# pyprob/pyprob

Hardware: AMD Instinct MI355X
Metric: ic_train_traces_per_sec (higher is better)
Workload: dtype f32; 1 GPU; GaussianUnknownMean IC training, offline traces resident in HBM, LSTM hidden=512, batch=1024 per GPU; traces_in_hbm=1000000, params=1643583, global_batch=1024, parallelism=dp1, optimizer=Adam lr=1e-3*sqrt(world), launch=one Python iteration per step (ICEngine.train_step), eager launches, prewarm_steps=5470, minibatches_resident=976, minibatch_walk=step i trains minibatch (i * 1) mod 976 of the resident dataset

## Files before the change

pyprob_amd/csrc/kernels.hip:

```cpp
#include "common.hpp"
#include "gather.hpp"
#include "head_math.hpp"
#include "aux_jobs.hpp"

#include <math.h>
#include <stdarg.h>
#include <stdlib.h>

#include <algorithm>
#include <vector>

namespace pp {

static thread_local char g_err[512] = "";
void set_error(const char* fmt, ...) {
    va_list ap;
    va_start(ap, fmt);
    vsnprintf(g_err, sizeof(g_err), fmt, ap);
    va_end(ap);
}
const char* last_error() { return g_err; }

constexpr int COLSUM_ROWS = 64;
constexpr int COLSUM_MAX_JOBS = 48;
// ... 712 lines not shown
    __builtin_amdgcn_fence(__ATOMIC_ACQUIRE, "wavefront");
}

template <int KIND, int NE>
__global__ __launch_bounds__(256) void head_tail_kernel(const TailJobs jobs, int64_t lda1, int hid, int K,
                                                        const float* __restrict__ value,
                                                        const float* __restrict__ prior, int rows_per_wave,
                                                        float grad_scale, float* __restrict__ lp_out, int64_t lddy,
                                                        int64_t lddz, float* __restrict__ loss_acc,
                                                        int32_t* __restrict__ nonfinite, long long* __restrict__ dbg) {
    extern __shared__ __attribute__((aligned(16))) float tail_lds[];
    const TailJob& jb = jobs.j[blockIdx.y];
    const int n = jb.n;
    if ((int)blockIdx.x * 4 * rows_per_wave >= n) return;
    const float* __restrict__ A1 = jb.A1;
    const float* __restrict__ W2 = jb.W2;
    const float* __restrict__ b2 = jb.b2;
    const int32_t* __restrict__ rows = jb.rows;
    float* __restrict__ DY = jb.DY;
    float* __restrict__ dZ1 = jb.dZ1;
#define PP_STAMP(k) do { if (dbg && threadIdx.x == 0 && blockIdx.y == 0 && blockIdx.x == 0) dbg[(k)] = clock64(); } while (0)
    PP_STAMP(0);
    const int tid = threadIdx.x, lane = tid & 63, wave = tid >> 6;
    const int n_out = 3 * K;
    const int hid4 = (hid + 3) & ~3;
    const int ws = hid | 1;
    const int wtot = n_out * ws, wtot4 = (wtot + 3) & ~3;
    float* const w2s = tail_lds;
    float* const a1s = tail_lds + wtot4 + wave * hid4;
    float* const ys = tail_lds + wtot4 + 4 * hid4 + wave * 128;
    float* const dys = ys + 64;
    if (ws == hid && (reinterpret_cast<uintptr_t>(W2) & 15) == 0) {
        const f32x4* __restrict__ src = reinterpret_cast<const f32x4*>(W2);
        const int n4 = wtot >> 2;
        for (int base = tid; base < n4; base += 256 * 8) {
            f32x4 v[8];
#pragma unroll
            for (int u = 0; u < 8; ++u) v[u] = src[min(base + 256 * u, n4 - 1)];
#pragma unroll
            for (int u = 0; u < 8; ++u)
                if (base + 256 * u < n4) *reinterpret_cast<f32x4*>(w2s + 4 * (base + 256 * u)) = v[u];
        }
        for (int i = 4 * n4 + tid; i < wtot; i += 256) w2s[i] = W2[i];
    } else {
        const float inv = 1.0f / (float)ws;
        for (int base = tid; base < wtot; base += 256 * 16) {
            float v[16];
#pragma unroll
            for (int u = 0; u < 16; ++u) {
                const int i = min(base + 256 * u, wtot - 1);
                const int o = (int)(((float)i + 0.5f) * inv);
                const int j = i - o * ws;
                v[u] = W2[o * hid + min(j, hid - 1)];
            }
#pragma unroll
            for (int u = 0; u < 16; ++u)
                if (base + 256 * u < wtot) w2s[base + 256 * u] = v[u];
        }
    }
    const bool comp = lane < K;
    const float b2mu = comp ? b2[lane] : 0.0f, b2sd = comp ? b2[K + lane] : 0.0f, b2z = comp ? b2[2 * K + lane] : 0.0f;
    __syncthreads();
    PP_STAMP(1);
    const bool bwd = DY != nullptr;
    float loss_local = 0.f;
    bool bad_any = false;
    const int half = lane >> 5, l31 = lane & 31;
    const int jh = ((hid + 7) >> 3) << 2;
    const int jbeg = half * jh, jend = min(hid, jbeg + jh);
    int jc[NE];
#pragma unroll
    for (int e = 0; e < NE; ++e) jc[e] = min(lane + 64 * e, hid - 1);
    const int i0 = (blockIdx.x * 4 + wave) * rows_per_wave;
    for (int t = 0; t < rows_per_wave; ++t) {
        const int i = i0 + t;
        if (i >= n) break;
        const int r = rows ? rows[i] : i;
        float a1v[NE];
#pragma unroll
        for (int e = 0; e < NE; ++e) {
            const int j = lane + 64 * e;
            a1v[e] = j < hid ? A1[(int64_t)i * lda1 + j] : 0.0f;
            if (j < hid4) a1s[j] = a1v[e];
        }
        wave_lds_sync();
        PP_STAMP(2);
        for (int ob = 0; ob < n_out; ob += 32) {
            const int o = ob + l31;
            const float* __restrict__ wr = w2s + min(o, n_out - 1) * ws;
            float p0 = 0.0f, p1 = 0.0f, p2 = 0.0f, p3 = 0.0f;
            int j = jbeg;
#pragma unroll 4
            for (; j + 3 < jend; j += 4) {
                const f32x4 av = *reinterpret_cast<const f32x4*>(a1s + j);
                p0 += av[0] * wr[j];
                p1 += av[1] * wr[j + 1];
                p2 += av[2] * wr[j + 2];
                p3 += av[3] * wr[j + 3];
            }
            for (; j < jend; ++j) p0 += a1s[j] * wr[j];
            float acc = (p0 + p1) + (p2 + p3);
            acc += __shfl_xor(acc, 32, 64);
            if (half == 0 && o < n_out) ys[o] = acc;
        }
        wave_lds_sync();
        const float ymu = comp ? ys[lane] + b2mu : 0.0f;
        const float ysd = comp ? ys[K + lane] + b2sd : 0.0f;
        const float yz = comp ? ys[2 * K + lane] + b2z : -INFINITY;
        PP_STAMP(3);
        const float v = value[r], pa = prior[2 * r], pb = prior[2 * r + 1];
        const auto red_sum = [](float x) { return wave_sum(x); };
        const auto red_max = [](float x) { return wave_max(x); };
        LaneMixture hm;
        const float lp = lane_mixture_logprob<KIND>(comp, ymu, ysd, yz, v, pa, pb, red_sum, red_max, hm);
        PP_STAMP(4);
        if (lp_out && lane == 0) lp_out[r] = lp;
        const bool rescued = (lp == -INFINITY);
        const bool bad = !rescued && !isfinite(lp);
        bad_any |= bad;
        if (lane == 0) loss_local += rescued ? -kLogEps : -lp;
        if (!bwd) continue;
        const bool live = !(rescued || bad);
        float d0, d1, d2;
        lane_mixture_grad<KIND>(hm, comp, live, lp, pa, pb, grad_scale, red_sum, d0, d1, d2);
        if (comp) {
            float* dy = DY + (int64_t)i * lddy;
            dy[lane] = d0; dy[K + lane] = d1; dy[2 * K + lane] = d2;
            dys[lane] = d0; dys[K + lane] = d1; dys[2 * K + lane] = d2;
        }
        wave_lds_sync();
        PP_STAMP(5);
        float dz[NE];
#pragma unroll
        for (int e = 0; e < NE; ++e) dz[e] = 0.0f;
#pragma unroll 2
        for (int o = 0; o < n_out; ++o) {
            const float d = dys[o];
            const float* __restrict__ wr = w2s + o * ws;
#pragma unroll
            for (int e = 0; e < NE; ++e) dz[e] += d * wr[jc[e]];
        }
#pragma unroll
        for (int e = 0; e < NE; ++e) {
            const int j = lane + 64 * e;
            if (j < hid4) dZ1[(int64_t)i * lddz + j] = (j < hid && a1v[e] > 0.0f) ? dz[e] : 0.0f;
        }
        wave_lds_sync();
    }
    PP_STAMP(6);
    if (lane == 0 && loss_acc && loss_local != 0.0f) atomicAdd(loss_acc + 32 * ((blockIdx.x * 4 + wave + 7 * blockIdx.y) & 63), loss_local);
    if (bad_any && nonfinite && lane == 0) atomicOr(nonfinite, 1);
}

static size_t head_tail_lds_floats(int hid, int n_out) {
    const int hid4 = (hid + 3) & ~3;
    return (size_t)((n_out * (hid | 1) + 3) & ~3) + 4 * (size_t)hid4 + 4 * 128;
}

bool head_tail_supported(int kind, int hid, int n_out) {
    static const bool disabled = false;
    if (disabled) return false;
    if (kind != PP_HEAD_NORMAL_MIXTURE && kind != PP_HEAD_TRUNCNORMAL_MIXTURE && kind != PP_HEAD_POISSON_TN_MIXTURE) return false;
    if (n_out % 3 != 0 || n_out / 3 > MAXK || n_out / 3 < 1) return false;
    return hid >= 1 && hid <= 1024 && head_tail_lds_floats(hid, n_out) <= TAIL_LDS_FLOATS;
}

long long* g_timeline = nullptr;

template <int KIND, int NE>
static int head_tail_launch_ne(dim3 grid, size_t lds, hipStream_t st, const TailJobs& jobs, int64_t lda1, int hid, int K,
                               const float* value, const float* prior, int rpw, float gs, float* lp_out, int64_t lddy,
                               int64_t lddz, float* loss_acc, int32_t* nonfinite) {
    static thread_local bool configured = false;
    if (!configured) {
        hipError_t e = hipFuncSetAttribute((const void*)head_tail_kernel<KIND, NE>, hipFuncAttributeMaxDynamicSharedMemorySize,
                                           (int)(TAIL_LDS_FLOATS * sizeof(float)));
        if (e != hipSuccess) {
            set_error("head_tail: hipFuncSetAttribute failed: %s", hipGetErrorString(e));
            return (int)e;
        }
        configured = true;
    }
    hipLaunchKernelGGL((head_tail_kernel<KIND, NE>), grid, dim3(256), lds, st, jobs, lda1, hid, K, value, prior, rpw, gs, lp_out,
                       lddy, lddz, loss_acc, nonfinite, g_timeline);
    return 0;
}

template <int KIND>
static int head_tail_launch(int ne, dim3 grid, size_t lds, hipStream_t st, const TailJobs& jobs, int64_t lda1, int hid, int K,
                            const float* value, const float* prior, int rpw, float gs, float* lp_out, int64_t lddy,
                            int64_t lddz, float* loss_acc, int32_t* nonfinite) {
#define PP_TAIL(N) return head_tail_launch_ne<KIND, N>(grid, lds, st, jobs, lda1, hid, K, value, prior, rpw, gs, lp_out, lddy, \
                                                       lddz, loss_acc, nonfinite)
    if (ne <= 2) PP_TAIL(2);
    if (ne <= 4) PP_TAIL(4);
    if (ne <= 6) PP_TAIL(6);
    if (ne <= 8) PP_TAIL(8);
    if (ne <= 12) PP_TAIL(12);
    PP_TAIL(16);
#undef PP_TAIL
}

int head_tail_multi(int kind, const TailJob* jobs, int count, int64_t lda1, int hid, int n_out, const float* value,
                    const float* prior, float grad_scale, float* lp_out, int64_t lddy, int64_t lddz, float* loss_acc,
                    int32_t* nonfinite, hipStream_t st) {
    PP_CHECK_ARG(head_tail_supported(kind, hid, n_out), "head_tail: unsupported head shape");
    PP_CHECK_ARG(lda1 % 4 == 0 && lddz % 4 == 0, "head_tail: leading dimensions must be multiples of 4");
    const int ne = (hid + 63) / 64;
    const size_t lds = head_tail_lds_floats(hid, n_out) * sizeof(float);
    int i = 0;
    while (i < count) {
        TailJobs pack;
        int nj = 0, max_n = 0;
        for (; i < count && nj < TAIL_MAX_JOBS; ++i) {
            if (jobs[i].n <= 0) continue;
            PP_CHECK_ARG(jobs[i].A1 && jobs[i].W2 && jobs[i].b2 && (!jobs[i].DY || jobs[i].dZ1), "head_tail: bad job");
            pack.j[nj++] = jobs[i];
            max_n = std::max(max_n, jobs[i].n);
        }
        if (nj == 0) continue;
        const int rpw = std::max((max_n + 4 * 256 - 1) / (4 * 256), 1);
        dim3 grid(cdiv(max_n, 4 * rpw), nj);
        if (kind == PP_HEAD_NORMAL_MIXTURE)
            PP_TRY(head_tail_launch<0>(ne, grid, lds, st, pack, lda1, hid, n_out / 3, value, prior, rpw, grad_scale, lp_out, lddy,
                                       lddz, loss_acc, nonfinite));
        else if (kind == PP_HEAD_TRUNCNORMAL_MIXTURE)
            PP_TRY(head_tail_launch<1>(ne, grid, lds, st, pack, lda1, hid, n_out / 3, value, prior, rpw, grad_scale, lp_out, lddy,
                                       lddz, loss_acc, nonfinite));
        else
            PP_TRY(head_tail_launch<2>(ne, grid, lds, st, pack, lda1, hid, n_out / 3, value, prior, rpw, grad_scale, lp_out, lddy,
                                       lddz, loss_acc, nonfinite));
        PP_LAUNCH_CHECK("head_tail");
    }
    return 0;
}

__global__ void loss_finalize_kernel(const float* __restrict__ acc, const int32_t* __restrict__ flag, float inv_b,
                                     float* __restrict__ loss_out, int32_t* __restrict__ status_out) {
    float tot = 0.0f;
    for (int k = 0; k < 64; ++k) tot += acc[32 * k];
    const float l = tot * inv_b;
    loss_out[0] = l;
    if (status_out) status_out[0] = (flag[0] != 0 || !isfinite(l)) ? 1 : 0;
}

__global__ __launch_bounds__(256) void loss_rows_kernel(const float* __restrict__ lp, int n_rows, float inv_b,
                                                        const int32_t* __restrict__ flag, float* __restrict__ loss_out,
                                                        int32_t* __restrict__ status_out) {
    __shared__ double part[256];
    __shared__ int bad[256];
    double acc = 0.0;
    int b = 0;
    for (int r = threadIdx.x; r < n_rows; r += 256) {
        float l = lp[r];
        if (l == -INFINITY) l = kLogEps;
        if (!isfinite(l)) b = 1;
        acc -= (double)l;
    }
    part[threadIdx.x] = acc;
    bad[threadIdx.x] = b;
    __syncthreads();
    for (int s = 128; s > 0; s >>= 1) {
        if (threadIdx.x < s) {
            part[threadIdx.x] += part[threadIdx.x + s];
            bad[threadIdx.x] |= bad[threadIdx.x + s];
        }
        __syncthreads();
    }
    if (threadIdx.x == 0) {
        const float l = (float)(part[0] * (double)inv_b);
        loss_out[0] = l;
        if (status_out) status_out[0] = (bad[0] || (flag && flag[0] != 0) || !isfinite(l)) ? 1 : 0;
    }
}

int loss_from_rows(const float* lp, int n_rows, int n_traces, const int32_t* flag, float* loss_out, int32_t* status_out,
                   hipStream_t st) {
    hipLaunchKernelGGL(loss_rows_kernel, dim3(1), dim3(256), 0, st, lp, n_rows, 1.0f / (float)n_traces, flag, loss_out,
                       status_out);
    PP_LAUNCH_CHECK("loss_from_rows");
    return 0;
}

int loss_finalize(const float* acc, const int32_t* flag, int n_traces, float* loss_out, int32_t* status_out,
                  hipStream_t st) {
    hipLaunchKernelGGL(loss_finalize_kernel, dim3(1), dim3(1), 0, st, acc, flag, 1.0f / (float)n_traces, loss_out,
                       status_out);
    PP_LAUNCH_CHECK("loss_finalize");
    return 0;
}

constexpr int ADAM_TOP = 1024, ADAM_FIRST = 1025, ADAM_CHUNKS = 1026;
constexpr int ADAM_SEEN = 1027;

__global__ __launch_bounds__(256) void adam_kernel(float* __restrict__ P, float* __restrict__ Gr, float* __restrict__ M,
                                                   float* __restrict__ V, const int32_t* __restrict__ chunk_tensor,
                                                   int n_chunks, const float* __restrict__ active,
                                                   int32_t* __restrict__ tensor_step, int32_t* __restrict__ scratch, float lr,
                                                   float beta1, float beta2, float eps, float wd, float gscale,
                                                   int zero_grads, const int32_t* __restrict__ skip) {
    __shared__ float s_corr[2];
    const int b = blockIdx.x;
    const bool skipped = skip && skip[0] != 0;
    const int t = chunk_tensor[b];
    if (t < 0 || !(active[t] > 0.0f)) return;
    if (skipped) {
        if (zero_grads) *reinterpret_cast<f32x4*>(Gr + (int64_t)b * 1024 + threadIdx.x * 4) = f32x4{0.f, 0.f, 0.f, 0.f};
        return;
    }
    int32_t* const sc = scratch + (int64_t)t * PP_ADAM_SCRATCH;
    const int64_t o = (int64_t)b * 1024 + threadIdx.x * 4;
    const f32x4 g0 = *reinterpret_cast<const f32x4*>(Gr + o);
    __shared__ int s_seen;
    if (threadIdx.x == 0) s_seen = __atomic_load_n(sc + ADAM_SEEN, __ATOMIC_RELAXED);
    __syncthreads();
    const bool seen = s_seen != 0;
    bool idle = false;
    if (!seen && wd == 0.0f) {
        const bool zero = g0[0] == 0.0f && g0[1] == 0.0f && g0[2] == 0.0f && g0[3] == 0.0f;
        idle = __syncthreads_and(zero ? 1 : 0) != 0;
        if (!idle && threadIdx.x == 0) __atomic_store_n(sc + ADAM_SEEN, 1, __ATOMIC_RELAXED);
    } else if (!seen && threadIdx.x == 0) {
        __atomic_store_n(sc + ADAM_SEEN, 1, __ATOMIC_RELAXED);
    }
    f32x4 p = f32x4{0.f, 0.f, 0.f, 0.f}, m = p, v = p;
    if (!idle) {
        p = *reinterpret_cast<f32x4*>(P + o);
        m = *reinterpret_cast<f32x4*>(M + o);
        v = *reinterpret_cast<f32x4*>(V + o);
    }
    int step_old = 0, first = 0, chunks = 0;
    if (threadIdx.x == 0) {
        first = __atomic_load_n(sc + ADAM_FIRST, __ATOMIC_RELAXED) - 1;
        chunks = __atomic_load_n(sc + ADAM_CHUNKS, __ATOMIC_RELAXED);
        if (first < 0) {
            int lo = 0, hi = b;
            while (lo < hi) {
                const int mid = (lo + hi) >> 1;
                if (chunk_tensor[mid] < t) lo = mid + 1; else hi = mid;
            }
            int lo2 = b, hi2 = n_chunks;
            while (lo2 < hi2) {
                const int mid = (lo2 + hi2) >> 1;
                if (chunk_tensor[mid] <= t) lo2 = mid + 1; else hi2 = mid;
            }
            first = lo;
            chunks = lo2 - lo;
        }
        step_old = __atomic_load_n(tensor_step + t, __ATOMIC_RELAXED);
        const int step = step_old + 1;
        double p1 = 1.0, p2 = 1.0, q1 = (double)beta1, q2 = (double)beta2;
        for (int e = step; e > 0; e >>= 1) {
            if (e & 1) { p1 *= q1; p2 *= q2; }
            q1 *= q1;
            q2 *= q2;
        }
        const double bc1 = 1.0 - p1, bc2 = 1.0 - p2;
        s_corr[0] = (float)((double)lr / bc1);
        s_corr[1] = (float)(1.0 / sqrt(bc2));
    }
    __syncthreads();
    const float step_size = s_corr[0], inv_sqrt_bc2 = s_corr[1];
    const int k = (b - first) & 31;
    const int quota = (chunks - k + 31) >> 5;
    int ticket = -1;
    if (threadIdx.x == 0) ticket = atomicAdd(sc + 32 * k, 1);
    if (!idle) {
#pragma unroll
        for (int e = 0; e < 4; ++e) {
            float g = g0[e] * gscale;
            if (wd != 0.0f) g += wd * p[e];
            m[e] = beta1 * m[e] + (1.0f - beta1) * g;
            v[e] = beta2 * v[e] + (1.0f - beta2) * g * g;
            const float denom = sqrtf(v[e]) * inv_sqrt_bc2 + eps;
            p[e] -= step_size * (m[e] / denom);
        }
        *reinterpret_cast<f32x4*>(P + o) = p;
        *reinterpret_cast<f32x4*>(M + o) = m;
        *reinterpret_cast<f32x4*>(V + o) = v;
        if (zero_grads) *reinterpret_cast<f32x4*>(Gr + o) = f32x4{0.f, 0.f, 0.f, 0.f};
    }
    if (threadIdx.x == 0 && ticket == quota - 1) {
        __atomic_store_n(sc + 32 * k, 0, __ATOMIC_RELAXED);
        if (atomicAdd(sc + ADAM_TOP, 1) == min(chunks, 32) - 1) {
            __atomic_store_n(sc + ADAM_TOP, 0, __ATOMIC_RELAXED);
            __atomic_store_n(sc + ADAM_FIRST, first + 1, __ATOMIC_RELAXED);
            __atomic_store_n(sc + ADAM_CHUNKS, chunks, __ATOMIC_RELAXED);
            __atomic_store_n(tensor_step + t, step_old + 1, __ATOMIC_RELAXED);
        }
    }
}

int adam_step(float* params, float* grads, float* m, float* v, int64_t n_params, const int32_t* chunk_tensor,
              const float* active, int32_t* tensor_step, int32_t* scratch, int n_tensors, float lr, float beta1, float beta2,
              float eps, float wd, float gscale, int flags, const int32_t* skip, hipStream_t st) {
    PP_CHECK_ARG(params && grads && m && v && chunk_tensor && active && tensor_step && scratch, "pp_adam_step: null pointer");
    PP_CHECK_ARG(n_params % 1024 == 0, "pp_adam_step: n_params must be a multiple of 1024 (padded tensors)");
    if (n_tensors <= 0 || n_params == 0) return 0;
    const int n_chunks = (int)(n_params / 1024);
    hipLaunchKernelGGL(adam_kernel, dim3((unsigned)n_chunks), dim3(256), 0, st, params, grads, m, v, chunk_tensor, n_chunks,
                       active, tensor_step, scratch, lr, beta1, beta2, eps, wd, gscale, (flags & PP_ADAM_ZERO_GRADS) ? 1 : 0, skip);
    PP_LAUNCH_CHECK("pp_adam_step");
    return 0;
}

}
```

pyprob_amd/csrc/obs_embed.hip:

```cpp
#include "common.hpp"
#include "gather.hpp"
#include "obs_embed.hpp"
#include "panel.hpp"

#include <stdlib.h>

#include <algorithm>

namespace pp {

template <int NOBS>
__global__ __launch_bounds__(256) void obs_embed_fwd_kernel(const ObsFusedArgs ain, const float* __restrict__ P,
                                                            const float* __restrict__ obs, int n_traces,
                                                            int traces_per_wave, float* __restrict__ cat,
                                                            float* __restrict__ f1, float* __restrict__ E,
                                                            const RowBuild rbin, const AddrBias ab,
                                                            const PanelTranspose tr) {
    __shared__ float lds[10240];
    const ObsFusedArgs a = ain;
    const RowBuild rb = rbin;
    if (tr.n_blocks && (int)blockIdx.x >= tr.first_block) {
        panel_transpose_block(tr, (int)blockIdx.x - tr.first_block, lds);
        return;
    }
    if (ab.AB && (int)blockIdx.x >= ab.first_block) {
        addr_bias_block(ab, (int)blockIdx.x - ab.first_block, lds);
        return;
    }
    warm_kernargs((int)(sizeof(ObsFusedArgs) + sizeof(RowBuild) + sizeof(AddrBias) + sizeof(PanelTranspose)) + 64);
    const int tid = threadIdx.x, lane = tid & 63, wave = tid >> 6;
    if (rb.zero_small && blockIdx.x == 0)
        for (int q = tid; q < rb.n_small; q += 256) rb.zero_small[q] = 0.0f;
    obs_stage_all<NOBS>(a, P, lds, tid);
    __syncthreads();
    const int b0 = (blockIdx.x * 4 + wave) * traces_per_wave;
    for (int t = 0; t < traces_per_wave; ++t) {
        const int b = b0 + t;
        if (b >= n_traces) break;
        float h = 0.0f, c = 0.0f;
        int ci = 0, co = 0;
#pragma unroll
        for (int o = 0; o < NOBS; ++o) {
            if (o >= a.n_obs) break;
            const int jh = lane - a.hoff[o];
            const bool acth = jh >= 0 && jh < a.hid[o];
            if (acth) {
                const float* w = lds + a.l0[o].lds_w + jh * (a.in[o] + 1);
                float s = lds[a.l0[o].lds_b + jh];
                for (int i = 0; i < a.in[o]; ++i) s += w[i] * obs[(int64_t)b * a.width + ci + i];
                h = relu_keep_nan(s);
                a.obs_h[o][(int64_t)b * a.ohid_ld[o] + jh] = h;
            }
            ci += a.in[o];
        }
#pragma unroll
        for (int o = 0; o < NOBS; ++o) {
            if (o >= a.n_obs) break;
            const int jc = lane - co;
            const bool actc = jc >= 0 && jc < a.out[o];
            const float v = obs_dense(lds, a.l1[o], jc, actc, h, a.hoff[o]);
            if (actc) c = v;
            co += a.out[o];
        }
        const bool acte = lane < a.e_obs;
        if (acte) cat[(int64_t)b * a.e_ld + lane] = c;
        const float y1 = obs_dense(lds, a.f0, lane, acte, c, 0);
        if (acte) f1[(int64_t)b * a.e_ld + lane] = y1;
        const float y2 = obs_dense(lds, a.f1, lane, acte, y1, 0);
        if (acte) E[(int64_t)b * a.e_ld + lane] = y2;
        if (rb.X) {
            {
                const int c4 = rb.d.e_obs + rb.d.smp + rb.d.dtype + rb.d.addr;
                const int ad = rb.xcols > c4 ? rb.addr[b] : 0;
                float* xr = rb.X + (int64_t)b * rb.ldx;
                if (acte) xr[lane] = y2;
                for (int c = rb.d.e_obs + lane; c < rb.xcols; c += 64) xr[c] = gather_embedding_elem(rb.d, rb.params, rb.at, c, -1, 0.0f, ad);
                if (rb.zero_like) {
                    float* zr = rb.zero_like + (int64_t)b * rb.ldx;
                    for (int c = lane; c < rb.xcols; c += 64) zr[c] = 0.0f;
                }
            }
            for (int t = 1; t < rb.t_max; ++t) {
                const int r0 = rb.row_off[t];
                if (b >= rb.row_off[t + 1] - r0) break;
                const int r = r0 + b;
                const int pr = rb.prev_row[r];
                const int ap = pr < 0 ? -1 : rb.addr[pr];
                const float v = pr < 0 ? 0.0f : rb.value[pr];
                const int ad = rb.addr[r];
                float* xr = rb.X + (int64_t)r * rb.ldx;
                if (acte) xr[lane] = y2;
                for (int c = rb.d.e_obs + lane; c < rb.xcols; c += 64) xr[c] = gather_embedding_elem(rb.d, rb.params, rb.at, c, ap, v, ad);
                if (rb.zero_like) {
                    float* zr = rb.zero_like + (int64_t)r * rb.ldx;
                    for (int c = lane; c < rb.xcols; c += 64) zr[c] = 0.0f;
                }
            }
        }
    }
}

template <int NOBS>
__global__ __launch_bounds__(256) void obs_embed_dgrad_kernel(const ObsFusedArgs ain, const float* __restrict__ P,
                                                              int n_traces, int traces_per_wave,
                                                              const float* __restrict__ cat, const float* __restrict__ f1,
                                                              const float* __restrict__ dX, int64_t ldx,
                                                              const int32_t* __restrict__ row_off, int t_max,
                                                              const float* __restrict__ E, float* __restrict__ dE,
                                                              float* __restrict__ dF1, float* __restrict__ dCat,
                                                              float* const dHo0, int64_t dh_stride, int n_split,
                                                              int64_t split_stride) {
    __shared__ float lds[10240];
    warm_kernargs((int)sizeof(ObsFusedArgs) + 96);
    const ObsFusedArgs a = ain;
    const int tid = threadIdx.x, lane = tid & 63, wave = tid >> 6;
    int oh = -1, jh = 0;
    const float* my_h = nullptr;
    int64_t my_hld = 0;
#pragma unroll
    for (int o = 0; o < NOBS; ++o)
        if (o < a.n_obs && lane >= a.hoff[o] && lane < a.hoff[o] + a.hid[o]) {
            oh = o; jh = lane - a.hoff[o];
            my_h = a.obs_h[o]; my_hld = a.ohid_ld[o];
        }
    const bool acte = lane < a.e_obs;
    const int b0 = (blockIdx.x * 4 + wave) * traces_per_wave;
    auto load_dz2 = [&](int b) {
        float acc = 0.0f;
        if (acte) {
            acc = dX[(int64_t)b * ldx + lane];
            for (int z0 = 1; z0 < n_split; z0 += 8) {
                float pv[8];
#pragma unroll
                for (int u = 0; u < 8; ++u)
                    pv[u] = (z0 + u < n_split) ? dX[(int64_t)(z0 + u) * split_stride + (int64_t)b * ldx + lane] : 0.0f;
                acc += ((pv[0] + pv[1]) + (pv[2] + pv[3])) + ((pv[4] + pv[5]) + (pv[6] + pv[7]));
            }
            for (int t = 1; t < t_max; ++t) {
                const int r0 = row_off[t];
                if (b >= row_off[t + 1] - r0) break;
                acc += dX[(int64_t)(r0 + b) * ldx + lane];
            }
            acc = E[(int64_t)b * a.e_ld + lane] > 0.0f ? acc : 0.0f;
        }
        return acc;
    };
    float nx_dz2 = 0.f, nx_f1 = 0.f, nx_cat = 0.f, nx_h = 0.f;
    if (b0 < n_traces) {
        nx_dz2 = load_dz2(b0);
        nx_f1 = acte ? f1[(int64_t)b0 * a.e_ld + lane] : 0.0f;
        nx_cat = acte ? cat[(int64_t)b0 * a.e_ld + lane] : 0.0f;
        nx_h = oh >= 0 ? my_h[(int64_t)b0 * my_hld + jh] : 0.0f;
    }
    obs_stage_all<NOBS>(a, P, lds, tid);
    __syncthreads();
    for (int t = 0; t < traces_per_wave; ++t) {
        const int b = b0 + t;
        if (b >= n_traces) break;
        const float dz2 = nx_dz2, f1v = nx_f1, catv = nx_cat, hv = nx_h;
        if (t + 1 < traces_per_wave && b + 1 < n_traces) {
            const int bn = b + 1;
            nx_dz2 = load_dz2(bn);
            nx_f1 = acte ? f1[(int64_t)bn * a.e_ld + lane] : 0.0f;
            nx_cat = acte ? cat[(int64_t)bn * a.e_ld + lane] : 0.0f;
            nx_h = oh >= 0 ? my_h[(int64_t)bn * my_hld + jh] : 0.0f;
        }
        if (acte) dE[(int64_t)b * a.e_ld + lane] = dz2;
        float dz1 = obs_dense_t(lds, a.f1, lane, acte, dz2, 0);
        dz1 = f1v > 0.0f ? dz1 : 0.0f;
        if (acte) dF1[(int64_t)b * a.e_ld + lane] = dz1;
        float dzc = obs_dense_t(lds, a.f0, lane, acte, dz1, 0);
        dzc = catv > 0.0f ? dzc : 0.0f;
        if (acte) dCat[(int64_t)b * a.e_ld + lane] = dzc;
        float dh = 0.0f;
        int co = 0;
#pragma unroll
        for (int o = 0; o < NOBS; ++o) {
            if (o >= a.n_obs) break;
            const bool acth = (oh == o);
            const float d = obs_dense_t(lds, a.l1[o], jh, acth, dzc, co);
            if (acth) dh = d;
            co += a.out[o];
        }
        if (oh >= 0) dHo0[(int64_t)oh * dh_stride + (int64_t)b * my_hld + jh] = hv > 0.0f ? dh : 0.0f;
    }
}

static inline int64_t round4(int64_t x) { return (x + 3) & ~int64_t(3); }

bool obs_fused_supported(const pp_net* net) {
    if (net->e_obs > OBS_EMAX) return false;
    for (int o = 0; o < net->n_obs; ++o)
        if (net->obs_depth[o] != 0 && net->obs_depth[o] != 2) return false;
    int hsum = 0;
    for (int o = 0; o < net->n_obs; ++o) {
        if (net->obs_in[o] > OBS_INMAX || net->obs_hid[o] > OBS_HIDMAX || net->obs_hid[o] < 1) return false;
        hsum += net->obs_hid[o];
    }
    return hsum <= 64;
}

bool obs_fused_args(const pp_net* net, float* const* obs_h, ObsFusedArgs& a) {
    for (int o = 0; o < PP_MAX_OBS; ++o) a.obs_h[o] = o < net->n_obs ? obs_h[o] : nullptr;
    a.n_obs = net->n_obs;
    a.e_obs = net->e_obs;
    a.e_ld = round4(net->e_obs);
    int lds = 0, hoff = 0, width = 0;
    auto layer = [&](ObsLayer& L, int64_t w, int64_t b, int rows, int cols) {
        L.w_off = w; L.b_off = b; L.rows = rows; L.cols = cols;
        L.lds_w = lds; lds += rows * (cols + 1);
        L.lds_b = lds; lds += rows;
    };
    for (int o = 0; o < net->n_obs; ++o) {
        a.in[o] = net->obs_in[o]; a.hid[o] = net->obs_hid[o]; a.out[o] = net->obs_out[o];
        a.hoff[o] = hoff; hoff += a.hid[o];
        a.ohid_ld[o] = round4(a.hid[o]);
        width += a.in[o];
        layer(a.l0[o], net->obs_w0[o], net->obs_b0[o], a.hid[o], a.in[o]);
        layer(a.l1[o], net->obs_w1[o], net->obs_b1[o], a.out[o], a.hid[o]);
    }
    a.width = width;
    layer(a.f0, net->fin_w0, net->fin_b0, net->e_obs, net->e_obs);
    layer(a.f1, net->fin_w1, net->fin_b1, net->e_obs, net->e_obs);
    a.lds_total = lds;
    return lds + 1 <= 10240;
}

static int pick_traces_per_wave(int n, int target_blocks) {
    return std::max((n + 4 * target_blocks - 1) / (4 * target_blocks), 1);
}

int obs_embed_fwd_fused(const pp_net* net, const float* P, const float* obs, int n_traces, float* const* obs_h,
                        float* cat, float* f1, float* E, hipStream_t st, const RowBuild* rows, const AddrBias* bias,
                        const PanelTranspose* transpose) {
    ObsFusedArgs a;
    if (!obs_fused_supported(net) || !obs_fused_args(net, obs_h, a)) return PP_EINVAL;
    const int tpw = pick_traces_per_wave(n_traces, 256);
    RowBuild rb{};
    if (rows) rb = *rows;
    if (rb.X && rb.xcols <= 0) rb.xcols = rb.d.I;
    AddrBias ab{};
    int blocks = cdiv(n_traces, 4 * tpw);
    if (bias && bias->AB) {
        ab = *bias;
        ab.first_block = blocks;
        blocks += addr_bias_blocks(ab);
    }
    PanelTranspose tr{};
    if (transpose && transpose->n_blocks > 0) {
        tr = *transpose;
        tr.first_block = blocks;
        blocks += tr.n_blocks;
    }
#define PP_OBS_FWD(N) hipLaunchKernelGGL(obs_embed_fwd_kernel<N>, dim3(blocks), dim3(256), 0, st, a, P, obs, n_traces, tpw, cat, f1, E, rb, ab, tr)
    if (a.n_obs <= 1) PP_OBS_FWD(1);
    else if (a.n_obs <= 2) PP_OBS_FWD(2);
    else if (a.n_obs <= 4) PP_OBS_FWD(4);
    else PP_OBS_FWD(8);
#undef PP_OBS_FWD
    PP_LAUNCH_CHECK("obs_embed_fwd_fused");
    return 0;
}

int obs_embed_dgrad_fused(const pp_net* net, const float* P, int n_traces, float* const* obs_h, const float* cat,
                          const float* f1, const float* dX, int64_t ldx, const int32_t* row_off_dev, int t_max,
                          const float* E, float* dE, float* dF1, float* dCat, float* dHo0, int64_t dh_stride,
                          hipStream_t st, int n_split, int64_t split_stride) {
    ObsFusedArgs a;
    if (!obs_fused_supported(net) || !obs_fused_args(net, obs_h, a)) return PP_EINVAL;
    const int tpw = pick_traces_per_wave(n_traces, 256);
    const int nsp = n_split > 1 && t_max == 1 ? n_split : 1;
#define PP_OBS_BWD(N) hipLaunchKernelGGL(obs_embed_dgrad_kernel<N>, dim3(cdiv(n_traces, 4 * tpw)), dim3(256), 0, st, a, P, n_traces, tpw, cat, f1, dX, ldx, row_off_dev, t_max, E, dE, dF1, dCat, dHo0, dh_stride, nsp, split_stride)
    if (a.n_obs <= 1) PP_OBS_BWD(1);
    else if (a.n_obs <= 2) PP_OBS_BWD(2);
    else if (a.n_obs <= 4) PP_OBS_BWD(4);
    else PP_OBS_BWD(8);
#undef PP_OBS_BWD
    PP_LAUNCH_CHECK("obs_embed_dgrad_fused");
    return 0;
}

}
```

pyprob_amd/csrc/obs_embed.hpp:

```cpp
#pragma once
#include "common.hpp"

namespace pp {

constexpr int OBS_EMAX = 64;
constexpr int OBS_HIDMAX = 32;
constexpr int OBS_INMAX = 8;

struct ObsLayer {
    int64_t w_off, b_off;
    int rows, cols;
    int lds_w, lds_b;
};

struct ObsFusedArgs {
    int n_obs, e_obs, width;
    int in[PP_MAX_OBS], hid[PP_MAX_OBS], out[PP_MAX_OBS];
    int hoff[PP_MAX_OBS];
    ObsLayer l0[PP_MAX_OBS], l1[PP_MAX_OBS], f0, f1;
    int lds_total;
    int64_t ohid_ld[PP_MAX_OBS], e_ld;
    float* obs_h[PP_MAX_OBS];
};

__device__ __forceinline__ float bcast(float x, int idx) {
    return __int_as_float(__builtin_amdgcn_readlane(__float_as_int(x), idx));
}

template <int U, int NT = 256>
struct ObsStage {
    float v[U];
    __device__ __forceinline__ void load(const float* __restrict__ g, int n, int tid) {
#pragma unroll
        for (int u = 0; u < U; ++u) v[u] = g[min(tid + NT * u, n - 1)];
    }
    __device__ __forceinline__ void store(float* lds, int lds_w, int rows, int cols, int dummy, int tid) const {
        const int n = rows * cols;
        const float inv = 1.0f / (float)cols;
#pragma unroll
        for (int u = 0; u < U; ++u) {
            const int i = tid + NT * u;
            const int r = (int)(((float)i + 0.5f) * inv);
            const int off = lds_w + r * (cols + 1) + (i - r * cols);
            lds[i < n ? off : dummy] = v[u];
        }
    }
};

__device__ __forceinline__ float obs_dense_t(const float* lds, const ObsLayer& L, int col, bool act, float dz, int z_lane0) {
    const float* w = lds + L.lds_w + (act ? col : 0);
    const int ld = L.cols + 1;
    float s0 = 0.0f, s1 = 0.0f, s2 = 0.0f, s3 = 0.0f;
    int j = 0;
    for (; j + 8 <= L.rows; j += 8) {
        float wv[8];
#pragma unroll
        for (int q = 0; q < 8; ++q) wv[q] = w[(j + q) * ld];
        s0 += wv[0] * bcast(dz, z_lane0 + j) + wv[4] * bcast(dz, z_lane0 + j + 4);
        s1 += wv[1] * bcast(dz, z_lane0 + j + 1) + wv[5] * bcast(dz, z_lane0 + j + 5);
        s2 += wv[2] * bcast(dz, z_lane0 + j + 2) + wv[6] * bcast(dz, z_lane0 + j + 6);
        s3 += wv[3] * bcast(dz, z_lane0 + j + 3) + wv[7] * bcast(dz, z_lane0 + j + 7);
    }
    for (; j < L.rows; ++j) s0 += w[j * ld] * bcast(dz, z_lane0 + j);
    return act ? (s0 + s1) + (s2 + s3) : 0.0f;
}


template <int NOBS>
__device__ __forceinline__ void obs_stage_all(const ObsFusedArgs& a, const float* __restrict__ P, float* lds, int tid) {
    ObsStage<16> sf0, sf1;
    ObsStage<8> s1[NOBS];
    ObsStage<1> s0[NOBS];
    float bf0, bf1, b1[NOBS], b0[NOBS];
    sf0.load(P + a.f0.w_off, a.f0.rows * a.f0.cols, tid);
    sf1.load(P + a.f1.w_off, a.f1.rows * a.f1.cols, tid);
    bf0 = tid < a.f0.rows ? P[a.f0.b_off + tid] : 0.0f;
    bf1 = tid < a.f1.rows ? P[a.f1.b_off + tid] : 0.0f;
#pragma unroll
    for (int o = 0; o < NOBS; ++o) {
        if (o < a.n_obs) {
            s1[o].load(P + a.l1[o].w_off, a.l1[o].rows * a.l1[o].cols, tid);
            s0[o].load(P + a.l0[o].w_off, a.l0[o].rows * a.l0[o].cols, tid);
            b1[o] = tid < a.l1[o].rows ? P[a.l1[o].b_off + tid] : 0.0f;
            b0[o] = tid < a.l0[o].rows ? P[a.l0[o].b_off + tid] : 0.0f;
        }
    }
    const int dummy = a.lds_total;
    sf0.store(lds, a.f0.lds_w, a.f0.rows, a.f0.cols, dummy, tid);
    sf1.store(lds, a.f1.lds_w, a.f1.rows, a.f1.cols, dummy, tid);
    if (tid < a.f0.rows) lds[a.f0.lds_b + tid] = bf0;
    if (tid < a.f1.rows) lds[a.f1.lds_b + tid] = bf1;
#pragma unroll
    for (int o = 0; o < NOBS; ++o) {
        if (o < a.n_obs) {
            s1[o].store(lds, a.l1[o].lds_w, a.l1[o].rows, a.l1[o].cols, dummy, tid);
            s0[o].store(lds, a.l0[o].lds_w, a.l0[o].rows, a.l0[o].cols, dummy, tid);
            if (tid < a.l1[o].rows) lds[a.l1[o].lds_b + tid] = b1[o];
            if (tid < a.l0[o].rows) lds[a.l0[o].lds_b + tid] = b0[o];
        }
    }
}

__device__ __forceinline__ float obs_dense(const float* lds, const ObsLayer& L, int row, bool act, float x, int x_lane0) {
    const float* w = lds + L.lds_w + (act ? row : 0) * (L.cols + 1);
    float s0 = 0.0f, s1 = 0.0f, s2 = 0.0f, s3 = 0.0f;
    int k = 0;
    for (; k + 8 <= L.cols; k += 8) {
        float wv[8];
#pragma unroll
        for (int q = 0; q < 8; ++q) wv[q] = w[k + q];
        s0 += wv[0] * bcast(x, x_lane0 + k) + wv[4] * bcast(x, x_lane0 + k + 4);
        s1 += wv[1] * bcast(x, x_lane0 + k + 1) + wv[5] * bcast(x, x_lane0 + k + 5);
        s2 += wv[2] * bcast(x, x_lane0 + k + 2) + wv[6] * bcast(x, x_lane0 + k + 6);
        s3 += wv[3] * bcast(x, x_lane0 + k + 3) + wv[7] * bcast(x, x_lane0 + k + 7);
    }
    for (; k < L.cols; ++k) s0 += w[k] * bcast(x, x_lane0 + k);
    const float s = (s0 + s1) + (s2 + s3);
    return act ? relu_keep_nan(s + lds[L.lds_b + row]) : 0.0f;
}


template <int NOBS>
__device__ __forceinline__ float obs_forward_row(const ObsFusedArgs& a, const float* lds, const float* __restrict__ obs, int lane) {
    float h = 0.0f, c = 0.0f;
    int ci = 0, co = 0;
#pragma unroll
    for (int o = 0; o < NOBS; ++o) {
        if (o >= a.n_obs) break;
        const int jh = lane - a.hoff[o];
        const bool acth = jh >= 0 && jh < a.hid[o];
        if (acth) {
            const float* w = lds + a.l0[o].lds_w + jh * (a.in[o] + 1);
            float s = lds[a.l0[o].lds_b + jh];
            for (int i = 0; i < a.in[o]; ++i) s += w[i] * obs[ci + i];
            h = relu_keep_nan(s);
        }
        ci += a.in[o];
    }
#pragma unroll
    for (int o = 0; o < NOBS; ++o) {
        if (o >= a.n_obs) break;
        const int jc = lane - co;
        const bool actc = jc >= 0 && jc < a.out[o];
        const float v = obs_dense(lds, a.l1[o], jc, actc, h, a.hoff[o]);
        if (actc) c = v;
        co += a.out[o];
    }
    const bool acte = lane < a.e_obs;
    const float y1 = obs_dense(lds, a.f0, lane, acte, c, 0);
    return obs_dense(lds, a.f1, lane, acte, y1, 0);
}

bool obs_fused_args(const pp_net* net, float* const* obs_h, ObsFusedArgs& a);
bool obs_fused_supported(const pp_net* net);

}
```

Before: 15.66 million traces/s.

## Prefetch obs inputs and weight heads in obs embed; hoist Adam metadata loads

The obs embedding kernel now prefetches the next trace's observation inputs and address index, and the staged LDS weights for the next dense layer, while the current one computes. Weight/bias staging is restructured into branch-free loads, and a min-blocks launch bound is added. In Adam, the gradient and per-tensor metadata loads are issued before the early-exit checks so their latency overlaps. This adds register pressure, extra loads for blocks that exit early, and an occupancy hint that may force spills.

```diff
diff --git a/pyprob_amd/csrc/kernels.hip b/pyprob_amd/csrc/kernels.hip
--- a/pyprob_amd/csrc/kernels.hip
+++ b/pyprob_amd/csrc/kernels.hip
@@ -1038,17 +1038,26 @@
     __shared__ float s_corr[2];
     const int b = blockIdx.x;
     const bool skipped = skip && skip[0] != 0;
+    const int64_t o = (int64_t)b * 1024 + threadIdx.x * 4;
+    const f32x4 g0 = *reinterpret_cast<const f32x4*>(Gr + o);
     const int t = chunk_tensor[b];
-    if (t < 0 || !(active[t] > 0.0f)) return;
+    const int tc = max(t, 0);
+    const float act = active[tc];
+    int32_t* const sc = scratch + (int64_t)tc * PP_ADAM_SCRATCH;
+    int seen0 = 0, first = 0, chunks = 0, step_old = 0;
+    if (threadIdx.x == 0) {
+        seen0 = __atomic_load_n(sc + ADAM_SEEN, __ATOMIC_RELAXED);
+        first = __atomic_load_n(sc + ADAM_FIRST, __ATOMIC_RELAXED) - 1;
+        chunks = __atomic_load_n(sc + ADAM_CHUNKS, __ATOMIC_RELAXED);
+        step_old = __atomic_load_n(tensor_step + tc, __ATOMIC_RELAXED);
+    }
+    if (t < 0 || !(act > 0.0f)) return;
     if (skipped) {
         if (zero_grads) *reinterpret_cast<f32x4*>(Gr + (int64_t)b * 1024 + threadIdx.x * 4) = f32x4{0.f, 0.f, 0.f, 0.f};
         return;
     }
-    int32_t* const sc = scratch + (int64_t)t * PP_ADAM_SCRATCH;
-    const int64_t o = (int64_t)b * 1024 + threadIdx.x * 4;
-    const f32x4 g0 = *reinterpret_cast<const f32x4*>(Gr + o);
     __shared__ int s_seen;
-    if (threadIdx.x == 0) s_seen = __atomic_load_n(sc + ADAM_SEEN, __ATOMIC_RELAXED);
+    if (threadIdx.x == 0) s_seen = seen0;
     __syncthreads();
     const bool seen = s_seen != 0;
     bool idle = false;
@@ -1065,10 +1074,7 @@
         m = *reinterpret_cast<f32x4*>(M + o);
         v = *reinterpret_cast<f32x4*>(V + o);
     }
-    int step_old = 0, first = 0, chunks = 0;
     if (threadIdx.x == 0) {
-        first = __atomic_load_n(sc + ADAM_FIRST, __ATOMIC_RELAXED) - 1;
-        chunks = __atomic_load_n(sc + ADAM_CHUNKS, __ATOMIC_RELAXED);
         if (first < 0) {
             int lo = 0, hi = b;
             while (lo < hi) {
@@ -1083,7 +1089,6 @@
             first = lo;
             chunks = lo2 - lo;
         }
-        step_old = __atomic_load_n(tensor_step + t, __ATOMIC_RELAXED);
         const int step = step_old + 1;
         double p1 = 1.0, p2 = 1.0, q1 = (double)beta1, q2 = (double)beta2;
         for (int e = step; e > 0; e >>= 1) {
diff --git a/pyprob_amd/csrc/obs_embed.hip b/pyprob_amd/csrc/obs_embed.hip
--- a/pyprob_amd/csrc/obs_embed.hip
+++ b/pyprob_amd/csrc/obs_embed.hip
@@ -10,7 +10,7 @@
 namespace pp {
 
 template <int NOBS>
-__global__ __launch_bounds__(256) void obs_embed_fwd_kernel(const ObsFusedArgs ain, const float* __restrict__ P,
+__global__ __launch_bounds__(256, NOBS <= 4 ? 4 : 3) void obs_embed_fwd_kernel(const ObsFusedArgs ain, const float* __restrict__ P,
                                                             const float* __restrict__ obs, int n_traces,
                                                             int traces_per_wave, float* __restrict__ cat,
                                                             float* __restrict__ f1, float* __restrict__ E,
@@ -29,49 +29,48 @@
     }
     warm_kernargs((int)(sizeof(ObsFusedArgs) + sizeof(RowBuild) + sizeof(AddrBias) + sizeof(PanelTranspose)) + 64);
     const int tid = threadIdx.x, lane = tid & 63, wave = tid >> 6;
+    const int b0 = (blockIdx.x * 4 + wave) * traces_per_wave;
+    const ObsLaneIn li = obs_lane_in<NOBS>(a, lane);
+    const int c4 = rb.d.e_obs + rb.d.smp + rb.d.dtype + rb.d.addr;
+    const bool want_ad = rb.X && rb.xcols > c4;
+    float nx_x[OBS_INMAX];
+    int nx_ad = 0;
+    {
+        const int bc = min(b0, n_traces - 1);
+        obs_load_inputs(li, obs + (int64_t)bc * a.width, nx_x);
+        if (want_ad) nx_ad = rb.addr[bc];
+    }
     if (rb.zero_small && blockIdx.x == 0)
         for (int q = tid; q < rb.n_small; q += 256) rb.zero_small[q] = 0.0f;
     obs_stage_all<NOBS>(a, P, lds, tid);
     __syncthreads();
-    const int b0 = (blockIdx.x * 4 + wave) * traces_per_wave;
     for (int t = 0; t < traces_per_wave; ++t) {
         const int b = b0 + t;
         if (b >= n_traces) break;
-        float h = 0.0f, c = 0.0f;
-        int ci = 0, co = 0;
-#pragma unroll
-        for (int o = 0; o < NOBS; ++o) {
-            if (o >= a.n_obs) break;
-            const int jh = lane - a.hoff[o];
-            const bool acth = jh >= 0 && jh < a.hid[o];
-            if (acth) {
-                const float* w = lds + a.l0[o].lds_w + jh * (a.in[o] + 1);
-                float s = lds[a.l0[o].lds_b + jh];
-                for (int i = 0; i < a.in[o]; ++i) s += w[i] * obs[(int64_t)b * a.width + ci + i];
-                h = relu_keep_nan(s);
-                a.obs_h[o][(int64_t)b * a.ohid_ld[o] + jh] = h;
-            }
-            ci += a.in[o];
-        }
-#pragma unroll
-        for (int o = 0; o < NOBS; ++o) {
-            if (o >= a.n_obs) break;
-            const int jc = lane - co;
-            const bool actc = jc >= 0 && jc < a.out[o];
-            const float v = obs_dense(lds, a.l1[o], jc, actc, h, a.hoff[o]);
-            if (actc) c = v;
-            co += a.out[o];
-        }
+        float x[OBS_INMAX];
+#pragma unroll
+        for (int i = 0; i < OBS_INMAX; ++i) x[i] = nx_x[i];
+        const int ad0 = nx_ad;
+        if (t + 1 < traces_per_wave && b + 1 < n_traces) {
+            obs_load_inputs(li, obs + (int64_t)(b + 1) * a.width, nx_x);
+            if (want_ad) nx_ad = rb.addr[b + 1];
+        }
+        float h, c, y1;
+        const float y2 = obs_walk<NOBS>(a, lds, li, x, lane, h, c, y1);
         const bool acte = lane < a.e_obs;
-        if (acte) cat[(int64_t)b * a.e_ld + lane] = c;
-        const float y1 = obs_dense(lds, a.f0, lane, acte, c, 0);
-        if (acte) f1[(int64_t)b * a.e_ld + lane] = y1;
-        const float y2 = obs_dense(lds, a.f1, lane, acte, y1, 0);
-        if (acte) E[(int64_t)b * a.e_ld + lane] = y2;
+        if (li.oh >= 0) {
+#pragma unroll
+            for (int o = 0; o < NOBS; ++o)
+                if (o == li.oh) a.obs_h[o][(int64_t)b * a.ohid_ld[o] + li.jh] = h;
+        }
+        if (acte) {
+            cat[(int64_t)b * a.e_ld + lane] = c;
+            f1[(int64_t)b * a.e_ld + lane] = y1;
+            E[(int64_t)b * a.e_ld + lane] = y2;
+        }
         if (rb.X) {
             {
-                const int c4 = rb.d.e_obs + rb.d.smp + rb.d.dtype + rb.d.addr;
-                const int ad = rb.xcols > c4 ? rb.addr[b] : 0;
+                const int ad = ad0;
                 float* xr = rb.X + (int64_t)b * rb.ldx;
                 if (acte) xr[lane] = y2;
                 for (int c = rb.d.e_obs + lane; c < rb.xcols; c += 64) xr[c] = gather_embedding_elem(rb.d, rb.params, rb.at, c, -1, 0.0f, ad);
diff --git a/pyprob_amd/csrc/obs_embed.hpp b/pyprob_amd/csrc/obs_embed.hpp
--- a/pyprob_amd/csrc/obs_embed.hpp
+++ b/pyprob_amd/csrc/obs_embed.hpp
@@ -32,11 +32,11 @@
     float v[U];
     __device__ __forceinline__ void load(const float* __restrict__ g, int n, int tid) {
 #pragma unroll
-        for (int u = 0; u < U; ++u) v[u] = g[min(tid + NT * u, n - 1)];
+        for (int u = 0; u < U; ++u) v[u] = g[max(min(tid + NT * u, n - 1), 0)];
     }
     __device__ __forceinline__ void store(float* lds, int lds_w, int rows, int cols, int dummy, int tid) const {
         const int n = rows * cols;
-        const float inv = 1.0f / (float)cols;
+        const float inv = 1.0f / (float)max(cols, 1);
 #pragma unroll
         for (int u = 0; u < U; ++u) {
             const int i = tid + NT * u;
@@ -71,84 +71,160 @@
     ObsStage<16> sf0, sf1;
     ObsStage<8> s1[NOBS];
     ObsStage<1> s0[NOBS];
-    float bf0, bf1, b1[NOBS], b0[NOBS];
+    ObsStage<1> bf0, bf1, b1[NOBS], b0[NOBS];
+    ObsLayer l1[NOBS], l0[NOBS];
+#pragma unroll
+    for (int o = 0; o < NOBS; ++o) {
+        const bool on = o < a.n_obs;
+        l1[o] = a.l1[o]; l0[o] = a.l0[o];
+        if (!on) {
+            l1[o].w_off = l1[o].b_off = l0[o].w_off = l0[o].b_off = 0;
+            l1[o].rows = l1[o].cols = l0[o].rows = l0[o].cols = 0;
+            l1[o].lds_w = l1[o].lds_b = l0[o].lds_w = l0[o].lds_b = 0;
+        }
+    }
+    const int dummy = a.lds_total;
     sf0.load(P + a.f0.w_off, a.f0.rows * a.f0.cols, tid);
     sf1.load(P + a.f1.w_off, a.f1.rows * a.f1.cols, tid);
-    bf0 = tid < a.f0.rows ? P[a.f0.b_off + tid] : 0.0f;
-    bf1 = tid < a.f1.rows ? P[a.f1.b_off + tid] : 0.0f;
-#pragma unroll
-    for (int o = 0; o < NOBS; ++o) {
-        if (o < a.n_obs) {
-            s1[o].load(P + a.l1[o].w_off, a.l1[o].rows * a.l1[o].cols, tid);
-            s0[o].load(P + a.l0[o].w_off, a.l0[o].rows * a.l0[o].cols, tid);
-            b1[o] = tid < a.l1[o].rows ? P[a.l1[o].b_off + tid] : 0.0f;
-            b0[o] = tid < a.l0[o].rows ? P[a.l0[o].b_off + tid] : 0.0f;
-        }
-    }
-    const int dummy = a.lds_total;
+    bf0.load(P + a.f0.b_off, a.f0.rows, tid);
+    bf1.load(P + a.f1.b_off, a.f1.rows, tid);
+    constexpr bool ONE_TRIP = NOBS <= 2;
+    if (ONE_TRIP) {
+#pragma unroll
+        for (int o = 0; o < NOBS; ++o) {
+            s1[o].load(P + l1[o].w_off, l1[o].rows * l1[o].cols, tid);
+            s0[o].load(P + l0[o].w_off, l0[o].rows * l0[o].cols, tid);
+            b1[o].load(P + l1[o].b_off, l1[o].rows, tid);
+            b0[o].load(P + l0[o].b_off, l0[o].rows, tid);
+        }
+    }
     sf0.store(lds, a.f0.lds_w, a.f0.rows, a.f0.cols, dummy, tid);
     sf1.store(lds, a.f1.lds_w, a.f1.rows, a.f1.cols, dummy, tid);
-    if (tid < a.f0.rows) lds[a.f0.lds_b + tid] = bf0;
-    if (tid < a.f1.rows) lds[a.f1.lds_b + tid] = bf1;
-#pragma unroll
-    for (int o = 0; o < NOBS; ++o) {
-        if (o < a.n_obs) {
-            s1[o].store(lds, a.l1[o].lds_w, a.l1[o].rows, a.l1[o].cols, dummy, tid);
-            s0[o].store(lds, a.l0[o].lds_w, a.l0[o].rows, a.l0[o].cols, dummy, tid);
-            if (tid < a.l1[o].rows) lds[a.l1[o].lds_b + tid] = b1[o];
-            if (tid < a.l0[o].rows) lds[a.l0[o].lds_b + tid] = b0[o];
-        }
-    }
-}
-
-__device__ __forceinline__ float obs_dense(const float* lds, const ObsLayer& L, int row, bool act, float x, int x_lane0) {
+    lds[tid < a.f0.rows ? a.f0.lds_b + tid : dummy] = bf0.v[0];
+    lds[tid < a.f1.rows ? a.f1.lds_b + tid : dummy] = bf1.v[0];
+#pragma unroll
+    for (int o = 0; o < NOBS; ++o) {
+        if (!ONE_TRIP) {
+            s1[o].load(P + l1[o].w_off, l1[o].rows * l1[o].cols, tid);
+            s0[o].load(P + l0[o].w_off, l0[o].rows * l0[o].cols, tid);
+            b1[o].load(P + l1[o].b_off, l1[o].rows, tid);
+            b0[o].load(P + l0[o].b_off, l0[o].rows, tid);
+        }
+        s1[o].store(lds, l1[o].lds_w, l1[o].rows, l1[o].cols, dummy, tid);
+        s0[o].store(lds, l0[o].lds_w, l0[o].rows, l0[o].cols, dummy, tid);
+        lds[tid < l1[o].rows ? l1[o].lds_b + tid : dummy] = b1[o].v[0];
+        lds[tid < l0[o].rows ? l0[o].lds_b + tid : dummy] = b0[o].v[0];
+    }
+}
+
+struct ObsDenseHead {
+    float w[8];
+    float bias;
+};
+__device__ __forceinline__ ObsDenseHead obs_dense_head(const float* lds, const ObsLayer& L, int row, bool act) {
+    const float* w = lds + L.lds_w + (act ? row : 0) * (L.cols + 1);
+    ObsDenseHead hd;
+#pragma unroll
+    for (int q = 0; q < 8; ++q) hd.w[q] = w[q];
+    hd.bias = lds[L.lds_b + (act ? row : 0)];
+    return hd;
+}
+
+__device__ __forceinline__ float obs_dense(const float* lds, const ObsLayer& L, int row, bool act, float x, int x_lane0,
+                                           const ObsDenseHead& hd) {
     const float* w = lds + L.lds_w + (act ? row : 0) * (L.cols + 1);
     float s0 = 0.0f, s1 = 0.0f, s2 = 0.0f, s3 = 0.0f;
+    float wv[8];
+#pragma unroll
+    for (int q = 0; q < 8; ++q) wv[q] = hd.w[q];
     int k = 0;
     for (; k + 8 <= L.cols; k += 8) {
-        float wv[8];
-#pragma unroll
-        for (int q = 0; q < 8; ++q) wv[q] = w[k + q];
+        float wn[8];
+#pragma unroll
+        for (int q = 0; q < 8; ++q) wn[q] = w[k + 8 + q];
         s0 += wv[0] * bcast(x, x_lane0 + k) + wv[4] * bcast(x, x_lane0 + k + 4);
         s1 += wv[1] * bcast(x, x_lane0 + k + 1) + wv[5] * bcast(x, x_lane0 + k + 5);
         s2 += wv[2] * bcast(x, x_lane0 + k + 2) + wv[6] * bcast(x, x_lane0 + k + 6);
         s3 += wv[3] * bcast(x, x_lane0 + k + 3) + wv[7] * bcast(x, x_lane0 + k + 7);
+#pragma unroll
+        for (int q = 0; q < 8; ++q) wv[q] = wn[q];
     }
     for (; k < L.cols; ++k) s0 += w[k] * bcast(x, x_lane0 + k);
     const float s = (s0 + s1) + (s2 + s3);
-    return act ? relu_keep_nan(s + lds[L.lds_b + row]) : 0.0f;
-}
-
-
-template <int NOBS>
-__device__ __forceinline__ float obs_forward_row(const ObsFusedArgs& a, const float* lds, const float* __restrict__ obs, int lane) {
-    float h = 0.0f, c = 0.0f;
-    int ci = 0, co = 0;
+    return act ? relu_keep_nan(s + hd.bias) : 0.0f;
+}
+
+struct ObsLaneIn {
+    int oh, jh, ci, n;
+};
+template <int NOBS>
+__device__ __forceinline__ ObsLaneIn obs_lane_in(const ObsFusedArgs& a, int lane) {
+    ObsLaneIn li{-1, 0, 0, 0};
+    int ci = 0;
 #pragma unroll
     for (int o = 0; o < NOBS; ++o) {
         if (o >= a.n_obs) break;
         const int jh = lane - a.hoff[o];
-        const bool acth = jh >= 0 && jh < a.hid[o];
-        if (acth) {
-            const float* w = lds + a.l0[o].lds_w + jh * (a.in[o] + 1);
-            float s = lds[a.l0[o].lds_b + jh];
-            for (int i = 0; i < a.in[o]; ++i) s += w[i] * obs[ci + i];
-            h = relu_keep_nan(s);
-        }
+        if (jh >= 0 && jh < a.hid[o]) li = ObsLaneIn{o, jh, ci, a.in[o]};
         ci += a.in[o];
     }
+    return li;
+}
+__device__ __forceinline__ void obs_load_inputs(const ObsLaneIn& li, const float* __restrict__ row, float (&x)[OBS_INMAX]) {
+#pragma unroll
+    for (int i = 0; i < OBS_INMAX; ++i) x[i] = row[li.ci + max(min(i, li.n - 1), 0)];
+}
+
+template <int NOBS>
+__device__ __forceinline__ float obs_walk(const ObsFusedArgs& a, const float* lds, const ObsLaneIn& li,
+                                          const float (&x)[OBS_INMAX], int lane, float& h_out, float& c_out, float& y1_out) {
+    const bool acte = lane < a.e_obs;
+    ObsDenseHead hd = obs_dense_head(lds, a.l1[0], lane, lane < a.out[0]);
+    float h = 0.0f, c = 0.0f;
+    if (li.oh >= 0) {
+        int lw = 0, lb = 0;
+#pragma unroll
+        for (int o = 0; o < NOBS; ++o)
+            if (o == li.oh) { lw = a.l0[o].lds_w; lb = a.l0[o].lds_b; }
+        const float* w = lds + lw + li.jh * (li.n + 1);
+        float s = lds[lb + li.jh], wi[OBS_INMAX];
+#pragma unroll
+        for (int i = 0; i < OBS_INMAX; ++i) wi[i] = w[min(i, li.n - 1)];
+#pragma unroll
+        for (int i = 0; i < OBS_INMAX; ++i) s = i < li.n ? s + wi[i] * x[i] : s;
+        h = relu_keep_nan(s);
+    }
+    int co = 0;
 #pragma unroll
     for (int o = 0; o < NOBS; ++o) {
         if (o >= a.n_obs) break;
         const int jc = lane - co;
         const bool actc = jc >= 0 && jc < a.out[o];
-        const float v = obs_dense(lds, a.l1[o], jc, actc, h, a.hoff[o]);
+        const int con = co + a.out[o];
+        ObsDenseHead nx;
+        if (o + 1 < NOBS && o + 1 < a.n_obs) {
+            const int jn = lane - con;
+            nx = obs_dense_head(lds, a.l1[o + 1 < NOBS ? o + 1 : o], jn, jn >= 0 && jn < a.out[o + 1 < NOBS ? o + 1 : o]);
+        } else {
+            nx = obs_dense_head(lds, a.f0, lane, acte);
+        }
+        const float v = obs_dense(lds, a.l1[o], jc, actc, h, a.hoff[o], hd);
         if (actc) c = v;
-        co += a.out[o];
-    }
-    const bool acte = lane < a.e_obs;
-    const float y1 = obs_dense(lds, a.f0, lane, acte, c, 0);
-    return obs_dense(lds, a.f1, lane, acte, y1, 0);
+        co = con;
+        hd = nx;
+    }
+    const ObsDenseHead h1 = obs_dense_head(lds, a.f1, lane, acte);
+    const float y1 = obs_dense(lds, a.f0, lane, acte, c, 0, hd);
+    h_out = h; c_out = c; y1_out = y1;
+    return obs_dense(lds, a.f1, lane, acte, y1, 0, h1);
+}
+
+template <int NOBS>
+__device__ __forceinline__ float obs_forward_row(const ObsFusedArgs& a, const float* lds, const float* __restrict__ obs, int lane) {
+    const ObsLaneIn li = obs_lane_in<NOBS>(a, lane);
+    float x[OBS_INMAX], h, c, y1;
+    obs_load_inputs(li, obs, x);
+    return obs_walk<NOBS>(a, lds, li, x, lane, h, c, y1);
 }
 
 bool obs_fused_args(const pp_net* net, float* const* obs_h, ObsFusedArgs& a);
```

Result: faster. 15.93 million traces/s (median of 6 runs) (+1.7%).
